# wyhuai/DDNM

Measured on NVIDIA H100. Metric: restored 256x256 images/sec @100 DDIM steps, higher is better.
Workload: dtype fp32

## Files before the change

### ddnm_b200/_lib.py

```python
import ctypes as C
import os

_HERE = os.path.dirname(os.path.abspath(__file__))
LIB_PATH = os.path.join(_HERE, "libddnm_b200.so")


class DDNMError(RuntimeError):
    pass


class SimpleCfg(C.Structure):
    _fields_ = [("ch", C.c_int), ("out_ch", C.c_int), ("n_levels", C.c_int), ("ch_mult", C.c_int * 8),
                ("num_res_blocks", C.c_int), ("n_attn_res", C.c_int), ("attn_res", C.c_int * 4),
                ("in_channels", C.c_int), ("resolution", C.c_int), ("groups", C.c_int), ("eps", C.c_float)]


class OpenAICfg(C.Structure):
    _fields_ = [("image_size", C.c_int), ("model_channels", C.c_int), ("num_res_blocks", C.c_int), ("n_levels", C.c_int),
                ("channel_mult", C.c_int * 8), ("n_attn_ds", C.c_int), ("attn_ds", C.c_int * 4),
                ("num_head_channels", C.c_int), ("out_channels", C.c_int), ("in_channels", C.c_int), ("groups", C.c_int),
                ("eps", C.c_float), ("num_classes", C.c_int), ("low_res", C.c_int), ("num_heads", C.c_int),
                ("num_heads_upsample", C.c_int), ("new_attention_order", C.c_int)]


# ... 85 lines not shown
    "ddnm_simplified_Ap": (C.c_int, [C.POINTER(SimpleDeg), _P, _I, _P, _P]),
    "ddnm_sample_simplified": (C.c_int, [_P, C.POINTER(SimpleDeg), C.POINTER(Schedule), _P, _P, _P, _I, _P, _P, _P]),
    "ddnm_hq_canvas": (C.c_int, [_P, _I, _I, _I, _I, _I, _P, _P]),
    "ddnm_hq_step": (C.c_int, [C.POINTER(SimpleDeg), _P, _P, _I, _P, _P, _I, _I, _P, _P, _P, C.POINTER(HqScalars), _I, _P, _P, _P, _P]),
    "ddnm_hq_undo": (C.c_int, [_P, _P, _F, _F, _LL, _P]),
    "ddnm_data_transform": (C.c_int, [_P, _LL, _P, _P, _I, _I, _P, _P]),
    "ddnm_inverse_data_transform": (C.c_int, [_P, _LL, _I, _I, _P, _P]),
    "ddnm_finish_images": (C.c_int, [_P, _P, _I, _I, _I, _I, _I, _I, _P, _P, _P, _P]),
    "ddnm_conv_tc": (C.c_int, [_P, _I, _I, _I, _I, _P, _P, _I, _I, _I, _P, _I, _P, _P, _P, _P]),
    "ddnm_conv_direct": (C.c_int, [_P, _I, _I, _I, _I, _P, _P, _I, _I, _I, _P, _P]),
    "ddnm_conv_stem_sr": (C.c_int, [_P, _P, _I, _I, _I, _I, _I, _I, _P, _P, _I, _P, _I, C.POINTER(_F), _P]),
    "ddnm_conv_tc_bench": (C.c_int, [_I, _I, _I, _I, _I, _I, _I, C.POINTER(_F), C.POINTER(_D)]),
    "ddnm_gnconv_chunk_bench": (C.c_int, [_I, _I, _I, _I, _I, _I, _I, C.POINTER(_F)]),
    "ddnm_groupnorm": (C.c_int, [_P, _I, _I, _I, _I, _I, _P, _P, _F, _I, _P, _P]),
    "ddnm_conv_gn_tc": (C.c_int, [_P, _I, _I, _I, _I, _I, _P, _P, _F, _I, _P, _P, _I, _P, _I, _P, _P, _P, _I, C.POINTER(_F), _P]),
    "ddnm_tc_debug_gn_fused": (C.c_int, [_I]),
    "ddnm_tc_debug_force_bn": (C.c_int, [_I]),
    "ddnm_tc_debug_deal": (C.c_int, [_I]),
    "ddnm_tc_debug_pair_dual": (C.c_int, [_I]),
    "ddnm_tc_debug_dual_mode": (C.c_int, [_I]),
    "ddnm_tc_debug_pair_mode": (C.c_int, [_I]),
    "ddnm_tc_debug_halo": (C.c_int, [_I]),
    "ddnm_tc_debug_pingpong": (C.c_int, [_I]),
}
EXPORTS = ["ddnm_last_error"] + list(_SIGS)


def lib():
    global _lib
    if _lib is None:
        if not os.path.exists(LIB_PATH):
            raise DDNMError(f"{LIB_PATH} not found: run `python -c 'import __graft_entry__ as g; g.build()'` first")
        L = C.CDLL(LIB_PATH)
        L.ddnm_last_error.restype = C.c_char_p
        L.ddnm_last_error.argtypes = []
        missing = [n for n in _SIGS if not hasattr(L, n)]
        if missing:
            raise DDNMError(f"{LIB_PATH} lacks symbols {missing}: stale build?")
        for name, (res, args) in _SIGS.items():
            fn = getattr(L, name)
            fn.restype, fn.argtypes = res, args
        _lib = L
    return _lib


def check(rc):
# ... 21 lines not shown
```

### ddnm_b200/csrc/api.cu

```cuda
#include "../../include/ddnm_b200.h"

#include <cstring>
#include <vector>

#include "api_util.cuh"
#include "engine.cuh"
#include "kernels.cuh"
#include "tc_gemm.cuh"

using namespace ddnm;

namespace ddnm {
thread_local std::string g_last_error;
}

extern "C" {

const char* ddnm_last_error(void) { return g_last_error.c_str(); }
int ddnm_version(void) { return 100; }

int ddnm_unet_simple_create(const ddnm_simple_cfg* c, int batch, void** handle) {
  DDNM_API_BEGIN
  DDNM_CHECK(c && handle, "null argument");
  SimpleCfg cfg;
// ... 471 lines not shown
  tc_debug_pair_mode(mode);
  DDNM_API_END
}
int ddnm_tc_debug_dual_mode(int mode) {
  DDNM_API_BEGIN
  tc_debug_dual_mode(mode);
  DDNM_API_END
}
int ddnm_tc_debug_pair_dual(int on) {
  DDNM_API_BEGIN
  tc_debug_pair_dual(on);
  DDNM_API_END
}
int ddnm_tc_debug_halo(int on) {
  DDNM_API_BEGIN
  tc_debug_halo(on);
  DDNM_API_END
}
int ddnm_tc_debug_pingpong(int on) {
  DDNM_API_BEGIN
  tc_debug_pingpong(on);
  DDNM_API_END
}
int ddnm_tc_debug_force_bn(int bn) {
  DDNM_API_BEGIN
  tc_debug_force_bn(bn);
  DDNM_API_END
}
}
```

### ddnm_b200/csrc/common.cuh

```cuda
#pragma once
#include <cuda_runtime.h>
#include <cuda_fp16.h>
#include <cuda.h>
#include <cstdint>
#include <cstdio>
#include <stdexcept>
#include <string>

namespace ddnm {

struct Error : std::runtime_error {
  using std::runtime_error::runtime_error;
};

#define DDNM_CHECK(cond, msg)                                                                     \
  do {                                                                                            \
    if (!(cond)) throw ::ddnm::Error(std::string(msg) + " [" #cond "] at " __FILE__ ":" + std::to_string(__LINE__)); \
  } while (0)

#define CUDA_CHECK(expr)                                                                          \
  do {                                                                                            \
    cudaError_t _e = (expr);                                                                      \
    if (_e != cudaSuccess)                                                                        \
      throw ::ddnm::Error(std::string("CUDA error: ") + cudaGetErrorString(_e) + " in " #expr " at " __FILE__ ":" + \
// ... 171 lines not shown
      "wgmma.mma_async.sync.aligned.m64n256k16.f32.f16.f16 "
      "{%0, %1, %2, %3, %4, %5, %6, %7, %8, %9, %10, %11, %12, %13, %14, %15, %16, %17, %18, %19, %20, %21, %22, %23, %24, %25, %26, %27, %28, %29, %30, %31, %32, %33, %34, %35, %36, %37, %38, %39, %40, %41, %42, %43, %44, %45, %46, %47, %48, %49, %50, %51, %52, %53, %54, %55, %56, %57, %58, %59, %60, %61, %62, %63, %64, %65, %66, %67, %68, %69, %70, %71, %72, %73, %74, %75, %76, %77, %78, %79, %80, %81, %82, %83, %84, %85, %86, %87, %88, %89, %90, %91, %92, %93, %94, %95, %96, %97, %98, %99, %100, %101, %102, %103, %104, %105, %106, %107, %108, %109, %110, %111, %112, %113, %114, %115, %116, %117, %118, %119, %120, %121, %122, %123, %124, %125, %126, %127}, "
      "%128, %129, p, 1, 1, 0, 0;\n\t}"
      : "+f"(d[0]), "+f"(d[1]), "+f"(d[2]), "+f"(d[3]), "+f"(d[4]), "+f"(d[5]), "+f"(d[6]), "+f"(d[7]), "+f"(d[8]), "+f"(d[9]), "+f"(d[10]), "+f"(d[11]), "+f"(d[12]), "+f"(d[13]), "+f"(d[14]), "+f"(d[15]), "+f"(d[16]), "+f"(d[17]), "+f"(d[18]), "+f"(d[19]), "+f"(d[20]), "+f"(d[21]), "+f"(d[22]), "+f"(d[23]), "+f"(d[24]), "+f"(d[25]), "+f"(d[26]), "+f"(d[27]), "+f"(d[28]), "+f"(d[29]), "+f"(d[30]), "+f"(d[31]), "+f"(d[32]), "+f"(d[33]), "+f"(d[34]), "+f"(d[35]), "+f"(d[36]), "+f"(d[37]), "+f"(d[38]), "+f"(d[39]), "+f"(d[40]), "+f"(d[41]), "+f"(d[42]), "+f"(d[43]), "+f"(d[44]), "+f"(d[45]), "+f"(d[46]), "+f"(d[47]), "+f"(d[48]), "+f"(d[49]), "+f"(d[50]), "+f"(d[51]), "+f"(d[52]), "+f"(d[53]), "+f"(d[54]), "+f"(d[55]), "+f"(d[56]), "+f"(d[57]), "+f"(d[58]), "+f"(d[59]), "+f"(d[60]), "+f"(d[61]), "+f"(d[62]), "+f"(d[63]), "+f"(d[64]), "+f"(d[65]), "+f"(d[66]), "+f"(d[67]), "+f"(d[68]), "+f"(d[69]), "+f"(d[70]), "+f"(d[71]), "+f"(d[72]), "+f"(d[73]), "+f"(d[74]), "+f"(d[75]), "+f"(d[76]), "+f"(d[77]), "+f"(d[78]), "+f"(d[79]), "+f"(d[80]), "+f"(d[81]), "+f"(d[82]), "+f"(d[83]), "+f"(d[84]), "+f"(d[85]), "+f"(d[86]), "+f"(d[87]), "+f"(d[88]), "+f"(d[89]), "+f"(d[90]), "+f"(d[91]), "+f"(d[92]), "+f"(d[93]), "+f"(d[94]), "+f"(d[95]), "+f"(d[96]), "+f"(d[97]), "+f"(d[98]), "+f"(d[99]), "+f"(d[100]), "+f"(d[101]), "+f"(d[102]), "+f"(d[103]), "+f"(d[104]), "+f"(d[105]), "+f"(d[106]), "+f"(d[107]), "+f"(d[108]), "+f"(d[109]), "+f"(d[110]), "+f"(d[111]), "+f"(d[112]), "+f"(d[113]), "+f"(d[114]), "+f"(d[115]), "+f"(d[116]), "+f"(d[117]), "+f"(d[118]), "+f"(d[119]), "+f"(d[120]), "+f"(d[121]), "+f"(d[122]), "+f"(d[123]), "+f"(d[124]), "+f"(d[125]), "+f"(d[126]), "+f"(d[127])
      : "l"(a_desc), "l"(b_desc), "r"(accumulate));
}
__device__ __forceinline__ uint32_t cluster_ctarank() {
  uint32_t r;
  asm volatile("mov.u32 %0, %%cluster_ctarank;" : "=r"(r));
  return r;
}
__device__ __forceinline__ uint32_t cluster_id_x() {
  uint32_t r;
  asm volatile("mov.u32 %0, %%clusterid.x;" : "=r"(r));
  return r;
}
__device__ __forceinline__ void cluster_sync_all() {
  asm volatile("barrier.cluster.arrive.release.aligned;" ::: "memory");
  asm volatile("barrier.cluster.wait.acquire.aligned;" ::: "memory");
}
__device__ __forceinline__ void mbar_arrive_cluster(uint32_t bar, uint32_t cta) {
  uint32_t remote;
  asm volatile("mapa.shared::cluster.u32 %0, %1, %2;" : "=r"(remote) : "r"(bar), "r"(cta));
  asm volatile("mbarrier.arrive.release.cluster.shared::cluster.b64 _, [%0];" ::"r"(remote) : "memory");
}
__device__ __forceinline__ void tma_load_3d_multicast(uint32_t dst, const void* tmap, uint32_t bar, int c0, int c1, int c2, uint16_t mask) {
  asm volatile(
      "cp.async.bulk.tensor.3d.shared::cluster.global.mbarrier::complete_tx::bytes.multicast::cluster [%0], [%1, {%3, %4, %5}], [%2], %6;" ::"r"(dst),
      "l"(tmap), "r"(bar), "r"(c0), "r"(c1), "r"(c2), "h"(mask)
      : "memory");
}
__device__ __forceinline__ void named_bar_sync(int id, int threads) { asm volatile("bar.sync %0, %1;" ::"r"(id), "r"(threads) : "memory"); }
template <int R>
__device__ __forceinline__ void setmaxnreg_dec() { asm volatile("setmaxnreg.dec.sync.aligned.u32 %0;" ::"n"(R)); }
template <int R>
__device__ __forceinline__ void setmaxnreg_inc() { asm volatile("setmaxnreg.inc.sync.aligned.u32 %0;" ::"n"(R)); }

__device__ __forceinline__ void stat_add(StatAcc* acc, float p) {
  const int bits = __float_as_int(p);
  int ex = (bits >> 23) & 0xff;
  unsigned long long m = (unsigned long long)(bits & 0x7fffff);
  if (ex) m |= 0x800000ull; else ex = 1;
  const int sh = ex - 150 + 48;
  unsigned long long lo = 0, hi = 0;
  if (sh >= 64) hi = m << min(sh - 64, 7);
  else if (sh > 0) { lo = m << sh; hi = sh > 40 ? m >> (64 - sh) : 0ull; }
  else if (sh > -24) lo = m >> (-sh);
// ... 43 lines not shown
```

### ddnm_b200/csrc/tc_gemm.cu

```cuda
#include "tc_gemm.cuh"

#include <cstdlib>

namespace ddnm {

static constexpr int BM = 128;
static constexpr int kConsumerThreads = 256;
static constexpr int kTcThreads = kConsumerThreads + 32;
static constexpr int BK = 64;
static constexpr int A_PLANE_BYTES = BM * BK * 2;
static constexpr int kGnMaxC = 512;

static constexpr int HALO_PLANE_BYTES = 17 * 1024;
static constexpr int HALO_UNITS = 2;

template <int BN, bool DUAL, bool HALO = false>
struct TcCfg {
  static constexpr int B_PLANE_BYTES = BN * BK * 2;
  static constexpr int A_UNIT_BYTES = 2 * HALO_PLANE_BYTES;
  static constexpr int A_RING_BYTES = HALO ? HALO_UNITS * A_UNIT_BYTES : 0;
  static constexpr int STAGE_BYTES = (HALO ? 0 : 2 * A_PLANE_BYTES) + 2 * B_PLANE_BYTES;
  static constexpr int STAGES = (HALO || BN == 64) ? 4 : 3;
  static constexpr int RING_BYTES = A_RING_BYTES + STAGES * STAGE_BYTES;
  static constexpr int PART_BYTES = 8 * BN * 8;
// ... 37 lines not shown
  y0 = ty * p.bh;
  n0 = tn * p.bn;
}

template <int STAGES>
struct TcBars {
  uint32_t base;
  __device__ uint32_t full(int s) const { return base + 8u * s; }
  __device__ uint32_t empty(int s) const { return base + 8u * (STAGES + s); }
  __device__ uint32_t a_full(int u) const { return base + 8u * (2 * STAGES + u); }
  __device__ uint32_t a_empty(int u) const { return base + 8u * (2 * STAGES + HALO_UNITS + u); }
  __device__ uint32_t turn(int w) const { return base + 8u * (2 * STAGES + 2 * HALO_UNITS + w); }
};

struct TcRing {
  uint32_t stage = 0, phase = 0;
  uint32_t aunit = 0, aphase = 0;
};

template <class Cfg, bool PAIR, bool GN, bool HALO>
__device__ __forceinline__ void tc_produce_tile(const CUtensorMap* tm_a0h, const CUtensorMap* tm_a0l, const CUtensorMap* tm_a1h,
                                                const CUtensorMap* tm_a1l, const CUtensorMap* tm_bh, const CUtensorMap* tm_bl,
                                                const TcParams& p, uint32_t smem_base, TcBars<Cfg::STAGES> bars, int tile, int kb_lo,
                                                int kb_hi, uint32_t rank, TcRing& r) {
  const int halo_r = p.mode0 == TAPS_UP2X2 ? 2 : 3;
  const int halo_w = p.bw + halo_r - 1;
  const bool lo = p.terms != 1;
  const uint32_t planes = lo ? 2u : 1u;
  const uint32_t stage_tx = (GN || HALO) ? planes * Cfg::B_PLANE_BYTES : (uint32_t)(lo ? Cfg::STAGE_BYTES : Cfg::STAGE_BYTES / 2);
  int n_idx, x0, y0, n0;
  tc_decode(p, tile, n_idx, x0, y0, n0);
  const int bz = p.b_batched == 1 ? n0 : 0;
  for (int kb = kb_lo; kb < kb_hi; ++kb) {
    int bkb = kb;
    if constexpr (HALO) {
      const int ua = kb / halo_r, dx = kb - ua * halo_r, dy = ua / p.cb0, cs = ua - dy * p.cb0;
      bkb = (dy * halo_r + dx) * p.cb0 + cs;
      if (dx == 0) {
        mbar_wait(bars.a_empty(r.aunit), r.aphase ^ 1u);
        const uint32_t ua_s = smem_base + r.aunit * Cfg::A_UNIT_BYTES;
        const uint32_t fa = bars.a_full(r.aunit);
        const int cy = y0 + dy - 1 + p.up_py, cx = x0 - 1 + p.up_px;
        mbar_expect_tx(fa, planes * (uint32_t)(halo_w * p.bh * 128));
        tma_load_4d(ua_s, tm_a0h, fa, cs * BK, cx, cy, n0);
        if (lo) tma_load_4d(ua_s + HALO_PLANE_BYTES, tm_a0l, fa, cs * BK, cx, cy, n0);
      }
      if (dx == halo_r - 1) {
        if (++r.aunit == HALO_UNITS) {
          r.aunit = 0;
          r.aphase ^= 1u;
        }
      }
    }
    mbar_wait(bars.empty(r.stage), r.phase ^ 1u);
    const uint32_t sa = smem_base + Cfg::A_RING_BYTES + r.stage * Cfg::STAGE_BYTES;
    const uint32_t sb = HALO ? sa : sa + 2 * A_PLANE_BYTES;
    const uint32_t fb = bars.full(r.stage);
    mbar_expect_tx(fb, stage_tx);
    if (GN || HALO) {
    } else if (kb < p.kb0) {
      const int tap = kb / p.cb0;
      const int c = (kb - tap * p.cb0) * BK;
      int cx = x0, cy = y0, cn = n0;
      if (p.mode0 == TAPS_3X3) {
        cy += tap / 3 - 1;
        cx += tap % 3 - 1;
      } else if (p.mode0 == TAPS_UP2X2) {
        cy += tap / 2 + p.up_py - 1;
        cx += tap % 2 + p.up_px - 1;
      } else if (p.mode0 == TAPS_3X3_S2) {
        const int dy = tap / 3, dx = tap % 3;
        cy += dy >> 1;
        cx += dx >> 1;
        cn += ((dy & 1) * 2 + (dx & 1)) * p.phase_stride;
      }
      tma_load_4d(sa, tm_a0h, fb, c, cx, cy, cn);
      if (lo) tma_load_4d(sa + A_PLANE_BYTES, tm_a0l, fb, c, cx, cy, cn);
    } else {
      const int c = (kb - p.kb0) * BK;
      tma_load_4d(sa, tm_a1h, fb, c, x0, y0, n0);
      if (lo) tma_load_4d(sa + A_PLANE_BYTES, tm_a1l, fb, c, x0, y0, n0);
    }
    if (PAIR) {
      constexpr int BN = Cfg::B_PLANE_BYTES / (BK * 2);
      const uint32_t half = rank * (BN / 2) * 128u;
      const int brow = n_idx * BN + (int)rank * (BN / 2);
      tma_load_3d_multicast(sb + half, tm_bh, fb, kb * BK, brow, 0, (uint16_t)3);
      if (lo) tma_load_3d_multicast(sb + Cfg::B_PLANE_BYTES + half, tm_bl, fb, kb * BK, brow, 0, (uint16_t)3);
    } else if (p.b_batched == 2) {
      constexpr int BN = Cfg::B_PLANE_BYTES / (BK * 2);
      tma_load_4d(sb, tm_bh, fb, kb * BK, n_idx * BN, y0, n0);
      if (lo) tma_load_4d(sb + Cfg::B_PLANE_BYTES, tm_bl, fb, kb * BK, n_idx * BN, y0, n0);
    } else {
      constexpr int BN = Cfg::B_PLANE_BYTES / (BK * 2);
      tma_load_3d(sb, tm_bh, fb, bkb * BK, n_idx * BN, bz);
      if (lo) tma_load_3d(sb + Cfg::B_PLANE_BYTES, tm_bl, fb, bkb * BK, n_idx * BN, bz);
    }
    if (++r.stage == Cfg::STAGES) {
      r.stage = 0;
      r.phase ^= 1u;
    }
  }
}

template <int BN, bool DUAL, bool NTAIL, int R>
__device__ __forceinline__ void tc_epilogue_rows(const TcParams& p, float (&d)[R], bool dual, int r0, int cq, int n_idx, int x0,
                                                 int y0, int n0, int split_off) {
  const int ppi = p.bw * p.bh;
  float* orow[2];
  const float* rrow[2];
  const float* crow[2];
// ... 336 lines not shown
            two_sum_acc(acc.x, acc.y, which ? pv.y : pv.x);
          }
          if (flush) {
            const int n = n0 + g;
            if (n < p.N) {
              StatAcc* dst = p.stats + ((size_t)n * p.st_ld + n_idx * BN + col) * 2 + which;
              stat_add(dst, acc.x);
              stat_add(dst, acc.y);
            }
            acc = make_float2(0.f, 0.f);
          }
        }
      }
      named_bar_sync(1, kConsumerThreads);
    }
  }
  }
  __syncwarp();
  if (PAIR) cluster_sync_all();
}

static constexpr int kPpThreads = 384;

template <int BN, bool HALO>
struct PpCfg {
  using Ring = TcCfg<BN, false, HALO>;
  static constexpr int PART_BYTES = 8 * BN * 8;
  static constexpr int RUN_BYTES = 2 * BN * 8;
  static constexpr int STAT_BYTES = PART_BYTES + RUN_BYTES;
  static constexpr int SMEM_BYTES = Ring::RING_BYTES + 1024  + 256  + 2 * STAT_BYTES;
  static_assert(SMEM_BYTES <= 227 * 1024, "shared memory capacity");
};

template <int BN, int TERMS, bool HALO, bool NTAIL>
__global__ void __launch_bounds__(kPpThreads, 1)
conv_tc_pingpong_kernel(const __grid_constant__ CUtensorMap tm_a0h, const __grid_constant__ CUtensorMap tm_a0l,
                        const __grid_constant__ CUtensorMap tm_a1h, const __grid_constant__ CUtensorMap tm_a1l,
                        const __grid_constant__ CUtensorMap tm_bh, const __grid_constant__ CUtensorMap tm_bl, const TcParams p) {
  static_assert(TERMS == 1 || TERMS == 3, "1 or 3 fp16 products per MAC");
  using Cfg = PpCfg<BN, HALO>;
  using Ring = typename Cfg::Ring;
  constexpr int STAGES = Ring::STAGES;
  extern __shared__ uint8_t smem_raw[];
  const uint32_t smem_base = (smem_u32(smem_raw) + 1023u) & ~1023u;
  const TcBars<STAGES> bars{smem_base + Ring::RING_BYTES};

  pdl_prologue();
  const int warp = threadIdx.x >> 5;
  const int lane = threadIdx.x & 31;
  const int KB = p.kb0 + p.kb1;
  const int n_units = p.tiles_x * p.tiles_y * p.tiles_n * p.n_tiles * p.split_k;
  const int n_workers = (int)gridDim.x, worker = (int)blockIdx.x;
  const int unit_begin = p.deal ? (int)((long long)worker * n_units / n_workers) : worker;
  const int unit_end = p.deal ? (int)((long long)(worker + 1) * n_units / n_workers) : n_units;
  const int unit_step = p.deal ? 1 : n_workers;
  auto k_lo = [&](int u) { return (int)((long long)(u % p.split_k) * KB / p.split_k); };
  auto k_hi = [&](int u) { return (int)((long long)(u % p.split_k + 1) * KB / p.split_k); };

  if (threadIdx.x == 0) {
    tma_prefetch_desc(&tm_a0h);
    tma_prefetch_desc(&tm_a0l);
    tma_prefetch_desc(&tm_bh);
    tma_prefetch_desc(&tm_bl);
    if (p.kb1) {
      tma_prefetch_desc(&tm_a1h);
      tma_prefetch_desc(&tm_a1l);
    }
    for (int s = 0; s < STAGES; ++s) {
      mbar_init(bars.full(s), 1);
      mbar_init(bars.empty(s), 4);
    }
    if (HALO) {
      for (int u = 0; u < HALO_UNITS; ++u) {
        mbar_init(bars.a_full(u), 1);
        mbar_init(bars.a_empty(u), 4);
      }
    }
    mbar_init(bars.turn(0), 4);
    mbar_init(bars.turn(1), 4);
    mbar_fence_init();
  }
  __syncthreads();

  if (warp < 4) {
    setmaxnreg_dec<40>();
    if (threadIdx.x == 0) {
      TcRing ring;
      for (int u = unit_begin; u < unit_end; u += unit_step)
        tc_produce_tile<Ring, false, false, HALO>(&tm_a0h, &tm_a0l, &tm_a1h, &tm_a1l, &tm_bh, &tm_bl, p, smem_base, bars,
                                                  u / p.split_k, k_lo(u), k_hi(u), 0u, ring);
    }
    return;
  }
  setmaxnreg_inc<232>();
  const int c = (warp >> 2) - 1;
  const int wq = warp & 3;
  const int tid = threadIdx.x - 128 * (c + 1);
  const int r0 = wq * 16 + (lane >> 2);
  const int cq = (lane & 3) * 2;
  const int halo_r = p.mode0 == TAPS_UP2X2 ? 2 : 3;
  const int halo_w = p.bw + halo_r - 1;
  const int units_per_tile = p.cb0 * halo_r;
  uint32_t halo_row_off[2];
#pragma unroll
  for (int f = 0; f < 2; ++f) halo_row_off[f] = (uint32_t)(((f * 64) / p.bw) * halo_w + (f * 64) % p.bw) * 128u;
  const int wpi = p.bw * p.bh >= 128 ? 8 : p.bw * p.bh / 16;
  uint8_t* stat_smem = smem_raw + (bars.base + 256u - smem_u32(smem_raw)) + c * Cfg::STAT_BYTES;
  float2* part = reinterpret_cast<float2*>(stat_smem);
  float2* run = reinterpret_cast<float2*>(stat_smem + Cfg::PART_BYTES);
  if (p.stats) {
    for (int i = tid; i < 2 * BN; i += 128) run[i] = make_float2(0.f, 0.f);
  }
  auto release = [&](int s) {
    if (lane == 0) mbar_arrive(bars.empty(s));
  };
  auto release_a = [&](uint32_t a) {
    if (lane == 0) mbar_arrive(bars.a_empty(a % HALO_UNITS));
  };
  uint32_t kpos = c ? (uint32_t)(k_hi(unit_begin) - k_lo(unit_begin)) : 0u;
  float d[2][BN / 2];
  int turn = 0;
  for (int u = unit_begin + c * unit_step; u < unit_end; u += 2 * unit_step, ++turn) {
    const int kb_lo = k_lo(u), kb_hi = k_hi(u);
    if (c == 1 || turn > 0) mbar_wait(bars.turn(c), (uint32_t)(c ? turn : turn - 1) & 1u);
    uint32_t stage = kpos % STAGES, phase = (kpos / STAGES) & 1u;
    const uint32_t a_done = (uint32_t)((2 * turn + c) * units_per_tile);
    int prev = -1;
    for (int kb = kb_lo; kb < kb_hi; ++kb) {
      const uint32_t sb = smem_base + Ring::A_RING_BYTES + stage * Ring::STAGE_BYTES;
      uint32_t a_base = sb;
      uint32_t a_frag1 = 64u * 128u;
      uint32_t a_plane = A_PLANE_BYTES;
      uint32_t a_unit = 0;
      bool a_first = false;
      if constexpr (HALO) {
        const int ua = halo_r == 3 ? (int)(__umulhi((uint32_t)kb, 0xAAAAAAABu) >> 1) : kb >> 1;
        const int dx = kb - ua * halo_r;
// ... 122 lines not shown
void tc_set_terms(int terms) {
  DDNM_CHECK(terms == 1 || terms == 3, "terms must be 1 or 3");
  g_terms = terms;
}
int tc_get_terms() { return g_terms; }
static int g_force_bn = 0;
void tc_debug_force_bn(int bn) {
  DDNM_CHECK(bn == 0 || bn == 64 || bn == 128, "BN must be 0 (heuristic), 64 or 128");
  g_force_bn = bn;
}
static int g_pair_mode = -1;
void tc_debug_pair_mode(int mode) {
  DDNM_CHECK(mode == -1 || mode == 0 || mode == 1, "pair mode must be -1 (default rule), 0 (off) or 1 (wherever legal)");
  g_pair_mode = mode;
}
static int g_dual_mode = 1;
void tc_debug_dual_mode(int mode) { g_dual_mode = mode; }
static int g_pair_dual = 1;
void tc_debug_pair_dual(int on) { g_pair_dual = on; }
static int g_halo_enable = [] { const char* v = std::getenv("DDNM_HALO"); return v && *v ? std::atoi(v) : 1; }();
void tc_debug_halo(int on) { g_halo_enable = on; }
static int g_pingpong_enable = [] { const char* v = std::getenv("DDNM_PINGPONG"); return v && *v ? std::atoi(v) : 1; }();
void tc_debug_pingpong(int on) { g_pingpong_enable = on; }
static int g_deal = -1;
void tc_debug_deal(int mode) {
  DDNM_CHECK(mode >= -1 && mode <= 1, "deal mode must be -1 (default rule), 0 (round-robin) or 1 (contiguous ranges)");
  g_deal = mode;
}

TcLaunch tc_make_launch(const SplitView& src0, int mode0, const SplitView* src1, const __half* w_hi, const __half* w_lo,
                        int w_batches, int Cout, const View& out, const float* chanadd, int ca_ld, const float* residual,
                        int ldr, float alpha, int num_sms, int res_mode) {
  TcLaunch L;
  TcParams& p = L.p;
  const int taps = (mode0 == TAPS_1X1) ? 1 : (mode0 == TAPS_UP2X2 ? 4 : 9);
  DDNM_CHECK(src0.C % BK == 0, "tensor-core conv needs Cin % 64 == 0");
  DDNM_CHECK(Cout % 64 == 0, "tensor-core conv needs Cout % 64 == 0");
  p.H = out.H; p.W = out.W; p.N = out.N;
  p.bw = out.W >= 128 ? 128 : out.W;
  DDNM_CHECK(128 % p.bw == 0 && out.W % p.bw == 0, "unsupported width for the 128-pixel tile");
  p.bh = std::min(out.H, 128 / p.bw);
  DDNM_CHECK(out.H % p.bh == 0 && 128 % (p.bw * p.bh) == 0, "unsupported height for the 128-pixel tile");
  p.bn = 128 / (p.bw * p.bh);
  p.tiles_x = out.W / p.bw;
  p.tiles_y = out.H / p.bh;
  p.tiles_n = cdiv(out.N, p.bn);
// ... 38 lines not shown
  const uint64_t ad[4] = {(uint64_t)src0.C, (uint64_t)src0.W, (uint64_t)src0.H, (uint64_t)src0.N};
  const uint32_t abox[4] = {(uint32_t)BK, (uint32_t)p.bw, (uint32_t)p.bh, (uint32_t)p.bn};
  L.a0h = make_map_f16(src0.hi, 4, ad, abox);
  L.a0l = make_map_f16(src0.lo, 4, ad, abox);
  L.halo = g_halo_enable != 0 && !L.pair && (mode0 == TAPS_3X3 || mode0 == TAPS_UP2X2) && p.bw % 64 == 0 && p.bn == 1 && !src1;
  if (L.halo) {
    const uint32_t hbox[4] = {(uint32_t)BK, (uint32_t)(p.bw + (mode0 == TAPS_UP2X2 ? 1 : 2)), (uint32_t)p.bh, 1u};
    L.hh = make_map_f16(src0.hi, 4, ad, hbox);
    L.hl = make_map_f16(src0.lo, 4, ad, hbox);
  }
  if (src1) {
    const uint64_t ad1[4] = {(uint64_t)src1->C, (uint64_t)src1->W, (uint64_t)src1->H, (uint64_t)src1->N};
    L.a1h = make_map_f16(src1->hi, 4, ad1, abox);
    L.a1l = make_map_f16(src1->lo, 4, ad1, abox);
  } else {
    L.a1h = L.a0h;
    L.a1l = L.a0l;
  }
  const int Ktot = (p.kb0 + p.kb1) * BK;
  const uint64_t bd[3] = {(uint64_t)Ktot, (uint64_t)Cout, (uint64_t)w_batches};
  const uint32_t bbox[3] = {(uint32_t)BK, (uint32_t)(L.pair ? L.BN / 2 : L.BN), 1u};
  L.bh = make_map_f16(w_hi, 3, bd, bbox);
  L.bl = make_map_f16(w_lo, 3, bd, bbox);
  const int total = p.tiles_x * p.tiles_y * p.tiles_n * p.n_tiles;
  L.grid = L.pair ? 2 * std::min(total / 2, num_sms / 2) : std::min(total, num_sms);
  const int units = L.pair ? total / 2 : total, workers = L.pair ? L.grid / 2 : L.grid;
  p.deal = g_deal >= 0 ? g_deal : (out.st != nullptr && p.n_tiles == 1 && units >= 2 * workers ? 1 : 0);
  if (p.n_tiles != 1) p.deal = 0;
  L.flops = 2.0 * (double)out.pixels() * Cout * Ktot;
  return L;
}

TcLaunch tc_make_up2_launch(const SplitView& src, const __half* w_hi, const __half* w_lo, int Cout, const View& out, const float* chanadd,
                            int ca_ld, int py, int px, int num_sms) {
  DDNM_CHECK(out.H == 2 * src.H && out.W == 2 * src.W && out.N == src.N, "upsample phase: output must be twice the source size");
  View lr = out;
  lr.H = src.H;
  lr.W = src.W;
  TcLaunch L = tc_make_launch(src, TAPS_UP2X2, nullptr, w_hi, w_lo, 1, Cout, lr, chanadd, ca_ld, nullptr, 0, 1.0f, num_sms, 0);
  TcParams& p = L.p;
  p.up_py = py;
  p.up_px = px;
  p.out = out.p + ((size_t)py * out.W + px) * out.ld;
  p.out_sx = 2LL * out.ld;
  p.out_sy = 2LL * out.W * out.ld;
  p.out_sn = (long long)out.H * out.W * out.ld;
// ... 55 lines not shown
  CUDA_CHECK(cudaGetLastError());
}

template <int BN>
static void launch_forms(const TcLaunch& L, cudaStream_t stream) {
  if (L.ntail) {
    if constexpr (BN == 64) {
      if (L.dual) launch_bn<BN, false, true, false, false, true>(L, stream);
      else launch_bn<BN, false, false, false, false, true>(L, stream);
      return;
    }
    throw Error("partial N tiles need BN = 64");
  }
  if (L.halo && L.dual) launch_bn<BN, false, true, false, true>(L, stream);
  else if (L.halo) launch_bn<BN, false, false, false, true>(L, stream);
  else if (L.gn && L.dual) launch_bn<BN, false, true, true>(L, stream);
  else if (L.gn) launch_bn<BN, false, false, true>(L, stream);
  else if (L.pair && L.dual) launch_bn<BN, true, true>(L, stream);
  else if (L.pair) launch_bn<BN, true, false>(L, stream);
  else if (L.dual) launch_bn<BN, false, true>(L, stream);
  else launch_bn<BN, false, false>(L, stream);
}

template <int BN, int TERMS, bool HALO, bool NTAIL = false>
static void launch_pingpong(const TcLaunch& L, cudaStream_t stream) {
  using Cfg = PpCfg<BN, HALO>;
  static bool attr_set[64] = {};
  if (first_use_on_device(attr_set))
    CUDA_CHECK(cudaFuncSetAttribute(conv_tc_pingpong_kernel<BN, TERMS, HALO, NTAIL>, cudaFuncAttributeMaxDynamicSharedMemorySize,
                                    Cfg::SMEM_BYTES));
  launch_pdl(conv_tc_pingpong_kernel<BN, TERMS, HALO, NTAIL>, dim3(L.grid), dim3(kPpThreads), (size_t)Cfg::SMEM_BYTES, stream, 1,
             HALO ? L.hh : L.a0h, HALO ? L.hl : L.a0l, L.a1h, L.a1l, L.bh, L.bl, L.p);
  CUDA_CHECK(cudaGetLastError());
}

template <int BN>
static void launch_pingpong_forms(const TcLaunch& L, cudaStream_t stream) {
  if (L.ntail) {
    if constexpr (BN == 64) {
      if (L.p.terms == 1) launch_pingpong<BN, 1, false, true>(L, stream);
      else launch_pingpong<BN, 3, false, true>(L, stream);
      return;
    }
    throw Error("partial N tiles need BN = 64");
  }
  if (L.p.terms == 1) {
    if (L.halo) launch_pingpong<BN, 1, true>(L, stream);
    else launch_pingpong<BN, 1, false>(L, stream);
  } else {
    if (L.halo) launch_pingpong<BN, 3, true>(L, stream);
    else launch_pingpong<BN, 3, false>(L, stream);
  }
}

static int g_gn_enable = [] { const char* v = std::getenv("DDNM_GN_FUSED"); return v && *v ? std::atoi(v) : 0; }();
void tc_debug_gn_fused(int on) { g_gn_enable = on; }

static bool gn_shape_ok(const View& x, const View* side, int Cout, const View& out) {
  if (out.W % 128 != 0 || x.C % BK != 0 || x.C > kGnMaxC || Cout % 64 != 0) return false;
  if (x.H != out.H || x.W != out.W || x.N != out.N) return false;
  if (x.ld % 4 != 0 || ((uintptr_t)x.p & 15) != 0) return false;
  if (side && (side->C % BK != 0 || side->ld % 4 != 0 || ((uintptr_t)side->p & 15) != 0 || side->H != out.H || side->W != out.W ||
               side->N != out.N))
    return false;
  return true;
}

bool tc_gn_eligible(const View& x, const View* side, int Cout, const View& out) { return g_gn_enable != 0 && gn_shape_ok(x, side, Cout, out); }

TcLaunch tc_make_gn_launch(const View& x, const GnAffine& gn, const View* side, const __half* w_hi, const __half* w_lo, int Cout,
                           const View& out, const float* chanadd, int ca_ld, const float* residual, int ldr, int num_sms) {
  DDNM_CHECK(gn_shape_ok(x, side, Cout, out), "fused GroupNorm convolution: unsupported shape");
  DDNM_CHECK(g_terms == 3, "the fused GroupNorm convolution implements the fp32-grade (3-term) arithmetic only");
  SplitView a;
  a.hi = const_cast<__half*>(w_hi);
// ... 45 lines not shown
```

### ddnm_b200/csrc/tc_gemm.cuh

```cuda
#pragma once
#include "common.cuh"

namespace ddnm {

enum TcTapMode : int {
  TAPS_3X3 = 0,
  TAPS_1X1 = 1,
  TAPS_3X3_S2 = 2,
  TAPS_UP2X2 = 3,
};

struct TcParams {
  int H, W, N;
  int bw, bh, bn;
  int tiles_x, tiles_y, tiles_n;
  int n_tiles;
  int mode0;
  int cb0, kb0;
  int kb1;
  int phase_stride;
  int up_py, up_px;
  int b_batched;
  long long out_sn, out_sy, out_sx;
  int Cout, ldc;
// ... 18 lines not shown
  const float* xs = nullptr;
  int xs_ld = 0;
  const StatAcc* st = nullptr;
  int st_ld = 0;
  const float* gamma = nullptr;
  const float* beta = nullptr;
  float eps = 0.f;
  int groups = 32;
  const float* ss = nullptr;
  int ss_ld = 0;
  int silu = 0, norm = 0;
};

struct TcLaunch {
  CUtensorMap a0h, a0l, a1h, a1l, bh, bl;
  CUtensorMap hh, hl;
  TcParams p;
  int BN = 128;
  bool pair = false;
  bool dual = false;
  bool gn = false;
  bool halo = false;
  bool pingpong = false;
  bool ntail = false;
  TcGnArgs g;
  int grid = 0;
  double flops = 0;
};

TcLaunch tc_make_launch(const SplitView& src0, int mode0, const SplitView* src1, const __half* w_hi, const __half* w_lo,
                        int w_batches, int Cout, const View& out, const float* chanadd, int ca_ld, const float* residual,
                        int ldr, float alpha, int num_sms, int res_mode = 0);
void tc_run(const TcLaunch& L, cudaStream_t stream);
TcLaunch tc_make_up2_launch(const SplitView& src, const __half* w_hi, const __half* w_lo, int Cout, const View& out, const float* chanadd,
                            int ca_ld, int py, int px, int num_sms);

struct GemmOperand {
  const __half* hi;
  const __half* lo;
  long long s_row, s_head, s_img;
};
TcLaunch tc_make_gemm_launch(const GemmOperand& A, const GemmOperand& B, int M, int N, int K, int heads, int images, float* out,
                             long long out_sn, long long out_sy, long long out_sx, float alpha, int num_sms);

struct GnAffine {
  const float* gamma = nullptr;
  const float* beta = nullptr;
  float eps = 1e-6f;
  int groups = 32;
  bool silu = true;
  const float* ss = nullptr;
  int ss_ld = 0;
};
bool tc_gn_eligible(const View& x, const View* side, int Cout, const View& out);
TcLaunch tc_make_gn_launch(const View& x, const GnAffine& gn, const View* side, const __half* w_hi, const __half* w_lo, int Cout,
                           const View& out, const float* chanadd, int ca_ld, const float* residual, int ldr, int num_sms);
void tc_debug_gn_fused(int on);

void tc_debug_force_bn(int bn);
void tc_debug_deal(int mode);
void tc_debug_pair_mode(int mode);
void tc_debug_dual_mode(int mode);
void tc_debug_pair_dual(int on);
void tc_debug_halo(int on);
void tc_debug_pingpong(int on);
void tc_set_terms(int terms);
int tc_get_terms();

}
```

### include/ddnm_b200.h

```cpp
#ifndef DDNM_B200_H
#define DDNM_B200_H

#ifdef __cplusplus
extern "C" {
#endif

const char* ddnm_last_error(void);
int ddnm_version(void);

typedef struct {
  int ch, out_ch, n_levels;
  int ch_mult[8];
  int num_res_blocks;
  int n_attn_res;
  int attn_res[4];
  int in_channels, resolution, groups;
  float eps;
} ddnm_simple_cfg;

int ddnm_unet_simple_create(const ddnm_simple_cfg* cfg, int batch, void** handle);

typedef struct {
  int image_size, model_channels, num_res_blocks, n_levels;
  int channel_mult[8];
// ... 142 lines not shown
                       unsigned char* out_u8_hwc, float* psnr, void* stream);

int ddnm_conv_tc(const float* x, int N, int H, int W, int Cin, const float* w, const float* bias, int Cout, int mode, int up2,
                 const float* side_x, int CinSide, const float* side_w, const float* residual, float* out, void* stream);
int ddnm_conv_direct(const float* x, int N, int H, int W, int Cin, const float* w, const float* bias, int Cout, int mode, int up2,
                     float* out, void* stream);
int ddnm_conv_stem_sr(const float* x, const float* low_res, int N, int C, int H, int W, int h, int w, const float* weight,
                      const float* bias, int Cout, float* out, int iters, float* ms_per_iter, void* stream);
int ddnm_conv_tc_bench(int N, int H, int W, int Cin, int Cout, int mode, int iters, float* ms_per_iter, double* flops);
int ddnm_gnconv_chunk_bench(int N, int chunk, int H, int W, int Cin, int Cout, int iters, float* ms_per_pass);
int ddnm_groupnorm(const float* x, int N, int H, int W, int C, int groups, const float* gamma, const float* beta, float eps,
                   int silu, float* out, void* stream);
int ddnm_conv_gn_tc(const float* x, int N, int H, int W, int Cin, int groups, const float* gamma, const float* beta, float eps, int silu,
                    const float* w, const float* bias, int Cout, const float* side_x, int CinSide, const float* side_w,
                    const float* residual, float* out, int iters, float* ms_per_iter, void* stream);
int ddnm_tc_debug_gn_fused(int on);
int ddnm_tc_debug_force_bn(int bn);
int ddnm_tc_debug_deal(int mode);
int ddnm_tc_debug_pair_mode(int mode);
int ddnm_tc_debug_dual_mode(int mode);
int ddnm_tc_debug_pair_dual(int on);
int ddnm_tc_debug_halo(int on);
int ddnm_tc_debug_pingpong(int on);

#ifdef __cplusplus
}
#endif
#endif
```

Baseline: 3.129.

## Pair ping-pong conv CTAs in clusters to multicast shared weight tiles

Adds a 2-CTA cluster mode to the ping-pong tensor-core conv kernel. The two CTAs split each weight (B) tile load in half and multicast it to both. Empty barriers now take arrivals from both CTAs, and a ghost-production tail keeps the ring in step when the two CTAs have different unit counts. The aim is to halve weight traffic from L2/HBM per CTA. In exchange it adds cross-CTA synchronisation that couples the two CTAs' progress, and it falls back to single CTAs when cluster occupancy is too low. It also relaxes the cluster arrive from release.cluster semantics and fixes the multicast B coordinate to use bkb.

Result: faster. 3.230 (median of 6 runs) (+3.2%).

```diff
diff --git a/ddnm_b200/_lib.py b/ddnm_b200/_lib.py
--- a/ddnm_b200/_lib.py
+++ b/ddnm_b200/_lib.py
@@ -131,6 +131,7 @@
     "ddnm_tc_debug_pair_mode": (C.c_int, [_I]),
     "ddnm_tc_debug_halo": (C.c_int, [_I]),
     "ddnm_tc_debug_pingpong": (C.c_int, [_I]),
+    "ddnm_tc_debug_pp_pair": (C.c_int, [_I]),
 }
 EXPORTS = ["ddnm_last_error"] + list(_SIGS)
 
diff --git a/ddnm_b200/csrc/api.cu b/ddnm_b200/csrc/api.cu
--- a/ddnm_b200/csrc/api.cu
+++ b/ddnm_b200/csrc/api.cu
@@ -517,6 +517,11 @@
   tc_debug_pingpong(on);
   DDNM_API_END
 }
+int ddnm_tc_debug_pp_pair(int on) {
+  DDNM_API_BEGIN
+  tc_debug_pp_pair(on);
+  DDNM_API_END
+}
 int ddnm_tc_debug_force_bn(int bn) {
   DDNM_API_BEGIN
   tc_debug_force_bn(bn);
diff --git a/ddnm_b200/csrc/common.cuh b/ddnm_b200/csrc/common.cuh
--- a/ddnm_b200/csrc/common.cuh
+++ b/ddnm_b200/csrc/common.cuh
@@ -217,7 +217,7 @@
 __device__ __forceinline__ void mbar_arrive_cluster(uint32_t bar, uint32_t cta) {
   uint32_t remote;
   asm volatile("mapa.shared::cluster.u32 %0, %1, %2;" : "=r"(remote) : "r"(bar), "r"(cta));
-  asm volatile("mbarrier.arrive.release.cluster.shared::cluster.b64 _, [%0];" ::"r"(remote) : "memory");
+  asm volatile("mbarrier.arrive.shared::cluster.b64 _, [%0];" ::"r"(remote) : "memory");
 }
 __device__ __forceinline__ void tma_load_3d_multicast(uint32_t dst, const void* tmap, uint32_t bar, int c0, int c1, int c2, uint16_t mask) {
   asm volatile(
diff --git a/ddnm_b200/csrc/tc_gemm.cu b/ddnm_b200/csrc/tc_gemm.cu
--- a/ddnm_b200/csrc/tc_gemm.cu
+++ b/ddnm_b200/csrc/tc_gemm.cu
@@ -83,12 +83,13 @@
 __device__ __forceinline__ void tc_produce_tile(const CUtensorMap* tm_a0h, const CUtensorMap* tm_a0l, const CUtensorMap* tm_a1h,
                                                 const CUtensorMap* tm_a1l, const CUtensorMap* tm_bh, const CUtensorMap* tm_bl,
                                                 const TcParams& p, uint32_t smem_base, TcBars<Cfg::STAGES> bars, int tile, int kb_lo,
-                                                int kb_hi, uint32_t rank, TcRing& r) {
+                                                int kb_hi, uint32_t rank, TcRing& r, bool load_a = true) {
   const int halo_r = p.mode0 == TAPS_UP2X2 ? 2 : 3;
   const int halo_w = p.bw + halo_r - 1;
   const bool lo = p.terms != 1;
   const uint32_t planes = lo ? 2u : 1u;
-  const uint32_t stage_tx = (GN || HALO) ? planes * Cfg::B_PLANE_BYTES : (uint32_t)(lo ? Cfg::STAGE_BYTES : Cfg::STAGE_BYTES / 2);
+  const uint32_t stage_tx = (GN || HALO || !load_a) ? planes * Cfg::B_PLANE_BYTES
+                                                    : (uint32_t)(lo ? Cfg::STAGE_BYTES : Cfg::STAGE_BYTES / 2);
   int n_idx, x0, y0, n0;
   tc_decode(p, tile, n_idx, x0, y0, n0);
   const int bz = p.b_batched == 1 ? n0 : 0;
@@ -97,7 +98,7 @@
     if constexpr (HALO) {
       const int ua = kb / halo_r, dx = kb - ua * halo_r, dy = ua / p.cb0, cs = ua - dy * p.cb0;
       bkb = (dy * halo_r + dx) * p.cb0 + cs;
-      if (dx == 0) {
+      if (dx == 0 && load_a) {
         mbar_wait(bars.a_empty(r.aunit), r.aphase ^ 1u);
         const uint32_t ua_s = smem_base + r.aunit * Cfg::A_UNIT_BYTES;
         const uint32_t fa = bars.a_full(r.aunit);
@@ -118,7 +119,7 @@
     const uint32_t sb = HALO ? sa : sa + 2 * A_PLANE_BYTES;
     const uint32_t fb = bars.full(r.stage);
     mbar_expect_tx(fb, stage_tx);
-    if (GN || HALO) {
+    if (GN || HALO || !load_a) {
     } else if (kb < p.kb0) {
       const int tap = kb / p.cb0;
       const int c = (kb - tap * p.cb0) * BK;
@@ -146,8 +147,8 @@
       constexpr int BN = Cfg::B_PLANE_BYTES / (BK * 2);
       const uint32_t half = rank * (BN / 2) * 128u;
       const int brow = n_idx * BN + (int)rank * (BN / 2);
-      tma_load_3d_multicast(sb + half, tm_bh, fb, kb * BK, brow, 0, (uint16_t)3);
-      if (lo) tma_load_3d_multicast(sb + Cfg::B_PLANE_BYTES + half, tm_bl, fb, kb * BK, brow, 0, (uint16_t)3);
+      tma_load_3d_multicast(sb + half, tm_bh, fb, bkb * BK, brow, 0, (uint16_t)3);
+      if (lo) tma_load_3d_multicast(sb + Cfg::B_PLANE_BYTES + half, tm_bl, fb, bkb * BK, brow, 0, (uint16_t)3);
     } else if (p.b_batched == 2) {
       constexpr int BN = Cfg::B_PLANE_BYTES / (BK * 2);
       tma_load_4d(sb, tm_bh, fb, kb * BK, n_idx * BN, y0, n0);
@@ -530,6 +531,11 @@
 
 static constexpr int kPpThreads = 384;
 
+__device__ __forceinline__ int pp_worker(int cta, int T) {
+  const int k = cta >> 1;
+  return (k / T) * 2 * T + k % T + (cta & 1) * T;
+}
+
 template <int BN, bool HALO>
 struct PpCfg {
   using Ring = TcCfg<BN, false, HALO>;
@@ -540,12 +546,13 @@
   static_assert(SMEM_BYTES <= 227 * 1024, "shared memory capacity");
 };
 
-template <int BN, int TERMS, bool HALO, bool NTAIL>
+template <int BN, int TERMS, bool HALO, bool NTAIL, bool PAIR>
 __global__ void __launch_bounds__(kPpThreads, 1)
 conv_tc_pingpong_kernel(const __grid_constant__ CUtensorMap tm_a0h, const __grid_constant__ CUtensorMap tm_a0l,
                         const __grid_constant__ CUtensorMap tm_a1h, const __grid_constant__ CUtensorMap tm_a1l,
                         const __grid_constant__ CUtensorMap tm_bh, const __grid_constant__ CUtensorMap tm_bl, const TcParams p) {
   static_assert(TERMS == 1 || TERMS == 3, "1 or 3 fp16 products per MAC");
+  static_assert(!PAIR || !NTAIL, "CTA pairs share one weight matrix (no batched GEMMs)");
   using Cfg = PpCfg<BN, HALO>;
   using Ring = typename Cfg::Ring;
   constexpr int STAGES = Ring::STAGES;
@@ -558,12 +565,17 @@
   const int lane = threadIdx.x & 31;
   const int KB = p.kb0 + p.kb1;
   const int n_units = p.tiles_x * p.tiles_y * p.tiles_n * p.n_tiles * p.split_k;
-  const int n_workers = (int)gridDim.x, worker = (int)blockIdx.x;
+  const int n_workers = (int)gridDim.x, worker = PAIR ? pp_worker((int)blockIdx.x, p.n_tiles) : (int)blockIdx.x;
   const int unit_begin = p.deal ? (int)((long long)worker * n_units / n_workers) : worker;
   const int unit_end = p.deal ? (int)((long long)(worker + 1) * n_units / n_workers) : n_units;
   const int unit_step = p.deal ? 1 : n_workers;
   auto k_lo = [&](int u) { return (int)((long long)(u % p.split_k) * KB / p.split_k); };
   auto k_hi = [&](int u) { return (int)((long long)(u % p.split_k + 1) * KB / p.split_k); };
+  auto units_of = [&](int w) {
+    return p.deal ? (int)((long long)(w + 1) * n_units / n_workers) - (int)((long long)w * n_units / n_workers)
+                  : (n_units - w + n_workers - 1) / n_workers;
+  };
+  const int peer = worker + ((blockIdx.x & 1) ? -p.n_tiles : p.n_tiles);
 
   if (threadIdx.x == 0) {
     tma_prefetch_desc(&tm_a0h);
@@ -576,7 +588,7 @@
     }
     for (int s = 0; s < STAGES; ++s) {
       mbar_init(bars.full(s), 1);
-      mbar_init(bars.empty(s), 4);
+      mbar_init(bars.empty(s), PAIR ? 8 : 4);
     }
     if (HALO) {
       for (int u = 0; u < HALO_UNITS; ++u) {
@@ -588,15 +600,43 @@
     mbar_init(bars.turn(1), 4);
     mbar_fence_init();
   }
-  __syncthreads();
+  if (PAIR) cluster_sync_all();
+  else __syncthreads();
 
   if (warp < 4) {
     setmaxnreg_dec<40>();
     if (threadIdx.x == 0) {
       TcRing ring;
       for (int u = unit_begin; u < unit_end; u += unit_step)
-        tc_produce_tile<Ring, false, false, HALO>(&tm_a0h, &tm_a0l, &tm_a1h, &tm_a1l, &tm_bh, &tm_bl, p, smem_base, bars,
-                                                  u / p.split_k, k_lo(u), k_hi(u), 0u, ring);
+        tc_produce_tile<Ring, PAIR, false, HALO>(&tm_a0h, &tm_a0l, &tm_a1h, &tm_a1l, &tm_bh, &tm_bl, p, smem_base, bars,
+                                                 u / p.split_k, k_lo(u), k_hi(u), PAIR ? cluster_ctarank() : 0u, ring);
+      if constexpr (PAIR) {
+        const int peer_begin = p.deal ? (int)((long long)peer * n_units / n_workers) : peer;
+        const uint32_t g0 = (uint32_t)(units_of(worker) * KB);
+        uint32_t q = g0;
+        auto ghost_release = [&](uint32_t g) {
+          mbar_wait(bars.full(g % STAGES), (g / STAGES) & 1u);
+          for (int w = 0; w < 4; ++w) {
+            mbar_arrive(bars.empty(g % STAGES));
+            mbar_arrive_cluster(bars.empty(g % STAGES), cluster_ctarank() ^ 1u);
+          }
+        };
+        for (int j = units_of(worker); j < units_of(peer); ++j) {
+          for (int kb = 0; kb < KB; ++kb, ++q) {
+            if (q >= g0 + STAGES) ghost_release(q - STAGES);
+            tc_produce_tile<Ring, true, false, HALO>(&tm_a0h, &tm_a0l, &tm_a1h, &tm_a1l, &tm_bh, &tm_bl, p, smem_base, bars,
+                                                     peer_begin + j * unit_step, kb, kb + 1, cluster_ctarank(), ring, false);
+          }
+        }
+        for (uint32_t g = q >= g0 + STAGES ? q - STAGES : g0; g < q; ++g) ghost_release(g);
+        for (int s = 0; s < STAGES; ++s) {
+          mbar_wait(bars.empty(ring.stage), ring.phase ^ 1u);
+          if (++ring.stage == STAGES) {
+            ring.stage = 0;
+            ring.phase ^= 1u;
+          }
+        }
+      }
     }
     return;
   }
@@ -620,7 +660,10 @@
     for (int i = tid; i < 2 * BN; i += 128) run[i] = make_float2(0.f, 0.f);
   }
   auto release = [&](int s) {
-    if (lane == 0) mbar_arrive(bars.empty(s));
+    if (lane == 0) {
+      mbar_arrive(bars.empty(s));
+      if (PAIR) mbar_arrive_cluster(bars.empty(s), cluster_ctarank() ^ 1u);
+    }
   };
   auto release_a = [&](uint32_t a) {
     if (lane == 0) mbar_arrive(bars.a_empty(a % HALO_UNITS));
@@ -789,6 +832,8 @@
 void tc_debug_halo(int on) { g_halo_enable = on; }
 static int g_pingpong_enable = [] { const char* v = std::getenv("DDNM_PINGPONG"); return v && *v ? std::atoi(v) : 1; }();
 void tc_debug_pingpong(int on) { g_pingpong_enable = on; }
+static int g_pp_pair_enable = [] { const char* v = std::getenv("DDNM_PP_PAIR"); return v && *v ? std::atoi(v) : 1; }();
+void tc_debug_pp_pair(int on) { g_pp_pair_enable = on; }
 static int g_deal = -1;
 void tc_debug_deal(int mode) {
   DDNM_CHECK(mode >= -1 && mode <= 1, "deal mode must be -1 (default rule), 0 (round-robin) or 1 (contiguous ranges)");
@@ -873,6 +918,12 @@
   const uint32_t bbox[3] = {(uint32_t)BK, (uint32_t)(L.pair ? L.BN / 2 : L.BN), 1u};
   L.bh = make_map_f16(w_hi, 3, bd, bbox);
   L.bl = make_map_f16(w_lo, 3, bd, bbox);
+  L.pp_pair = g_pp_pair_enable != 0 && !L.pair && w_batches == 1 && mode0 != TAPS_UP2X2;
+  if (L.pp_pair) {
+    const uint32_t hbox[3] = {(uint32_t)BK, (uint32_t)(L.BN / 2), 1u};
+    L.bh2 = make_map_f16(w_hi, 3, bd, hbox);
+    L.bl2 = make_map_f16(w_lo, 3, bd, hbox);
+  }
   const int total = p.tiles_x * p.tiles_y * p.tiles_n * p.n_tiles;
   L.grid = L.pair ? 2 * std::min(total / 2, num_sms / 2) : std::min(total, num_sms);
   const int units = L.pair ? total / 2 : total, workers = L.pair ? L.grid / 2 : L.grid;
@@ -974,16 +1025,53 @@
   else launch_bn<BN, false, false>(L, stream);
 }
 
-template <int BN, int TERMS, bool HALO, bool NTAIL = false>
+template <int BN, int TERMS, bool HALO, bool NTAIL = false, bool PAIR = false>
 static void launch_pingpong(const TcLaunch& L, cudaStream_t stream) {
   using Cfg = PpCfg<BN, HALO>;
+  const auto kernel = conv_tc_pingpong_kernel<BN, TERMS, HALO, NTAIL, PAIR>;
   static bool attr_set[64] = {};
-  if (first_use_on_device(attr_set))
-    CUDA_CHECK(cudaFuncSetAttribute(conv_tc_pingpong_kernel<BN, TERMS, HALO, NTAIL>, cudaFuncAttributeMaxDynamicSharedMemorySize,
-                                    Cfg::SMEM_BYTES));
-  launch_pdl(conv_tc_pingpong_kernel<BN, TERMS, HALO, NTAIL>, dim3(L.grid), dim3(kPpThreads), (size_t)Cfg::SMEM_BYTES, stream, 1,
-             HALO ? L.hh : L.a0h, HALO ? L.hl : L.a0l, L.a1h, L.a1l, L.bh, L.bl, L.p);
+  static int max_clusters[64] = {};
+  if (first_use_on_device(attr_set)) {
+    CUDA_CHECK(cudaFuncSetAttribute(kernel, cudaFuncAttributeMaxDynamicSharedMemorySize, Cfg::SMEM_BYTES));
+    if (PAIR) {
+      cudaLaunchConfig_t cfg = {};
+      cudaLaunchAttribute at;
+      at.id = cudaLaunchAttributeClusterDimension;
+      at.val.clusterDim.x = 2;
+      at.val.clusterDim.y = 1;
+      at.val.clusterDim.z = 1;
+      cfg.gridDim = dim3(2);
+      cfg.blockDim = dim3(kPpThreads);
+      cfg.dynamicSmemBytes = Cfg::SMEM_BYTES;
+      cfg.attrs = &at;
+      cfg.numAttrs = 1;
+      int dev = 0;
+      CUDA_CHECK(cudaGetDevice(&dev));
+      CUDA_CHECK(cudaOccupancyMaxActiveClusters(&max_clusters[dev & 63], kernel, &cfg));
+    }
+  }
+  if (PAIR) {
+    int dev = 0;
+    CUDA_CHECK(cudaGetDevice(&dev));
+    if (L.grid / 2 > max_clusters[dev & 63]) {
+      launch_pingpong<BN, TERMS, HALO, NTAIL, false>(L, stream);
+      return;
+    }
+  }
+  launch_pdl(kernel, dim3(L.grid), dim3(kPpThreads), (size_t)Cfg::SMEM_BYTES, stream, PAIR ? 2 : 1, HALO ? L.hh : L.a0h,
+             HALO ? L.hl : L.a0l, L.a1h, L.a1l, PAIR ? L.bh2 : L.bh, PAIR ? L.bl2 : L.bl, L.p);
   CUDA_CHECK(cudaGetLastError());
+}
+
+template <int BN, bool PAIR>
+static void launch_pingpong_terms(const TcLaunch& L, cudaStream_t stream) {
+  if (L.p.terms == 1) {
+    if (L.halo) launch_pingpong<BN, 1, true, false, PAIR>(L, stream);
+    else launch_pingpong<BN, 1, false, false, PAIR>(L, stream);
+  } else {
+    if (L.halo) launch_pingpong<BN, 3, true, false, PAIR>(L, stream);
+    else launch_pingpong<BN, 3, false, false, PAIR>(L, stream);
+  }
 }
 
 template <int BN>
@@ -996,13 +1084,9 @@
     }
     throw Error("partial N tiles need BN = 64");
   }
-  if (L.p.terms == 1) {
-    if (L.halo) launch_pingpong<BN, 1, true>(L, stream);
-    else launch_pingpong<BN, 1, false>(L, stream);
-  } else {
-    if (L.halo) launch_pingpong<BN, 3, true>(L, stream);
-    else launch_pingpong<BN, 3, false>(L, stream);
-  }
+  if (L.pp_pair && L.p.split_k == 1 && L.grid % (2 * L.p.n_tiles) == 0 && (L.p.n_tiles == 1 || L.p.deal == 0))
+    launch_pingpong_terms<BN, true>(L, stream);
+  else launch_pingpong_terms<BN, false>(L, stream);
 }
 
 static int g_gn_enable = [] { const char* v = std::getenv("DDNM_GN_FUSED"); return v && *v ? std::atoi(v) : 0; }();
diff --git a/ddnm_b200/csrc/tc_gemm.cuh b/ddnm_b200/csrc/tc_gemm.cuh
--- a/ddnm_b200/csrc/tc_gemm.cuh
+++ b/ddnm_b200/csrc/tc_gemm.cuh
@@ -64,6 +64,8 @@
   bool gn = false;
   bool halo = false;
   bool pingpong = false;
+  bool pp_pair = false;
+  CUtensorMap bh2, bl2;
   bool ntail = false;
   TcGnArgs g;
   int grid = 0;
@@ -106,6 +108,7 @@
 void tc_debug_pair_dual(int on);
 void tc_debug_halo(int on);
 void tc_debug_pingpong(int on);
+void tc_debug_pp_pair(int on);
 void tc_set_terms(int terms);
 int tc_get_terms();
 
diff --git a/include/ddnm_b200.h b/include/ddnm_b200.h
--- a/include/ddnm_b200.h
+++ b/include/ddnm_b200.h
@@ -188,6 +188,7 @@
 int ddnm_tc_debug_pair_dual(int on);
 int ddnm_tc_debug_halo(int on);
 int ddnm_tc_debug_pingpong(int on);
+int ddnm_tc_debug_pp_pair(int on);
 
 #ifdef __cplusplus
 }
```
